# evandieren/AbstractBayesOpt.jl

Hardware: AMD Instinct MI355X
Metric: GP-update+acq-eval ms per BO step at N train pts x M candidates (lower is better)
Workload: dtype f64

## Files before the change

abstractbayesopt.jl_amd/_lib.py:

```python
import ctypes as C
import os

PKG = os.path.dirname(os.path.abspath(__file__))
LIB_PATH = os.path.join(PKG, "lib", "libabo_hip.so")
LIB_TEST_PATH = os.path.join(PKG, "lib", "libabo_hip_test.so")

ABO_OK, ABO_ENOTPD, ABO_EDIM, ABO_EINVAL, ABO_EHIP, ABO_ENOMEM = range(6)
HOST, DEVICE = 0, 1

EXPORTS = ["abo_create", "abo_set_contraction", "abo_create_grad", "abo_predict_grad", "abo_predict_grad_cov", "abo_retain", "abo_destroy", "abo_fit", "abo_append", "abo_append_grad", "abo_cand_create", "abo_cand_destroy",
           "abo_cand_refresh", "abo_cand_downdate", "abo_cand_save", "abo_cand_restore", "abo_cand_acq", "abo_cand_get", "abo_cand_point", "abo_cand_exclude", "abo_predict", "abo_acq", "abo_nlml", "abo_nlml_grad", "abo_nlml_grad_ard", "abo_lhs", "abo_score",
           "abo_get_factor", "abo_get_n", "abo_get_data", "abo_get_timings", "abo_get_prune_stats", "abo_get_prune_levels", "abo_last_error", "abo_abi_version", "abo_pool_trim",
           "abo_mgpu_create", "abo_mgpu_clone", "abo_mgpu_destroy", "abo_mgpu_info", "abo_mgpu_get", "abo_mgpu_fit",
           "abo_mgpu_predict", "abo_mgpu_acq", "abo_mgpu_acq_lhs", "abo_mgpu_append", "abo_mgpu_cand_create",
           "abo_mgpu_cand_create_lhs", "abo_mgpu_cand_refresh", "abo_mgpu_cand_destroy", "abo_mgpu_cand_acq",
           "abo_mgpu_cand_qei", "abo_refine", "abo_optimize_acquisition", "abo_mgpu_optimize_acquisition", "abo_fit_acq", "abo_mgpu_create_grad", "abo_mgpu_append_grad", "abo_mgpu_cand_get", "abo_acq_terms", "abo_acq_lhs", "abo_refine_terms",
           "abo_optimize_acquisition_terms", "abo_mgpu_optimize_acquisition_terms",
           "abo_set_qei_block", "abo_cand_qei", "abo_cand_qei_begin", "abo_cand_qei_top", "abo_cand_qei_block", "abo_cand_qei_pick",
           "abo_cand_qei_end", "abo_cand_qei_has", "abo_cand_qei_stats", "abo_mgpu_cand_qei_stats", "abo_cand_qei_eligible", "abo_fill_distance",
           "abo_update", "abo_mgpu_update", "abo_cand_qei_mc",
           "abo_paths_create", "abo_paths_destroy", "abo_paths_eval", "abo_paths_eval_cand", "abo_paths_stats_get",
           "abo_paths_append", "abo_paths_attach", "abo_paths_detach", "abo_paths_top", "abo_paths_values", "abo_paths_append_stats_get",
           "abo_score_mes", "abo_acq_mes", "abo_cand_acq_mes", "abo_refine_mes", "abo_optimize_acquisition_mes",
           "abo_loo", "abo_loo_grad", "abo_predict_cov", "abo_remove"]
TEST_EXPORTS = ["abo_test_gemm_nt", "abo_test_kappa", "abo_test_oz_plan", "abo_test_oz_contract", "abo_test_acq_grad",
                "abo_test_acq_grad_terms", "abo_test_prune_plan", "abo_test_prune_force", "abo_test_prune_levels", "abo_test_prune_plan_levels", "abo_test_prune_bounds", "abo_test_prune_mean",
                "abo_test_kappa_tail", "abo_test_prune_tail32", "abo_test_prune_reuse", "abo_test_prune_reused", "abo_test_prune_head32", "abo_test_bound_head32", "abo_test_kappa_tail32", "abo_test_prune_bound_moduli", "abo_test_prune_bound_plan", "abo_test_oz_contract_bound", "abo_test_acq_partials", "abo_test_mes_partials", "abo_test_acq_grad_mes",
                "abo_test_gemm_args", "abo_test_gemm_path", "abo_test_gemm_swz_q", "abo_test_gemm_swz_map", "abo_test_qei_pass", "abo_test_splitk_reduce",
                "abo_test_var_gemm", "abo_test_kgen", "abo_test_cand_newcol",
                "abo_test_chol_diag", "abo_test_chol_panel", "abo_test_trtri_batched", "abo_test_chol_blocked", "abo_test_trmv",
                "abo_test_nlml_terms", "abo_test_append",
                "abo_test_topk_plan", "abo_test_topk", "abo_test_prune_compact", "abo_test_prune_min_scatter", "abo_test_prune_map",
                "abo_test_finalize", "abo_test_cand_gemv", "abo_test_downdate", "abo_test_grad_cov", "abo_test_gather_points",
                "abo_test_pick_record", "abo_test_score",
                "abo_test_oz_rowscale", "abo_test_oz_quant", "abo_test_oz_gemm", "abo_test_oz_crt", "abo_test_oz_modpack", "abo_test_oz_tickets"]
TOPK_PATH_NONE, TOPK_PATH_SMALL, TOPK_PATH_SLICES, TOPK_PATH_ARGMAX, TOPK_PATH_BLOCKSORT = -1, 0, 1, 2, 3
PRUNE_REL, PRUNE_ABS, PRUNE_ABS_LOGEI = 2.0 ** -30, 2.0 ** -1022, 2.0 ** -30
GEMM_PATH_TILED, GEMM_PATH_SWIZZLED, GEMM_PATH_SMALL, GEMM_PATH_SKINNY, GEMM_PATH_SPLITK = range(5)
K_FULL, K_A_LOWER, K_A_UPPER, K_B_LOWER, K_B_UPPER = range(5)
ABI_VERSION = 7
CONTRACT_AUTO, CONTRACT_FP64, CONTRACT_INT8 = 0, 1, 2
UPDATE_SHARED, UPDATE_APPENDED, UPDATE_REFIT = 0, 1, 2
UPDATE_PATHS = {UPDATE_SHARED: "shared", UPDATE_APPENDED: "appended", UPDATE_REFIT: "refit"}
REMOVE_REMOVED, REMOVE_REFIT = 0, 1
REMOVE_PATHS = {REMOVE_REMOVED: "removed", REMOVE_REFIT: "refit"}


class AboParams(C.Structure):
    _fields_ = [("family", C.c_int32), ("device", C.c_int32), ("ell", C.c_double), ("sigma_f2", C.c_double),
                ("noise_var", C.c_double), ("mean_c", C.c_double), ("jitter", C.c_double),
                ("n_max", C.c_int64), ("chunk", C.c_int64)]


class AboTimings(C.Structure):
    _fields_ = [(n, C.c_double) for n in ("fit_kernel_matrix_ms", "fit_cholesky_ms", "fit_inverse_ms",
                                          "fit_alpha_ms", "fit_total_ms", "acq_kxz_ms", "acq_var_gemm_ms",
                                          "acq_finalize_ms", "acq_topk_ms", "acq_total_ms")] + \
               [("var_gemm_launches", C.c_int64), ("var_gemm_flop", C.c_double), ("downdate_ms", C.c_double),
                ("downdate_bytes", C.c_double), ("contraction_engine", C.c_int64), ("oz_nmod", C.c_int64)] + \
               [(n, C.c_double) for n in ("oz_prepare_ms", "oz_quant_ms", "oz_gemm_ms", "oz_crt_ms", "oz_gemm_ops", "refine_ms")] + \
               [("refine_starts", C.c_int64), ("refine_evals", C.c_int64), ("downdate_from_chain", C.c_int64),
# ... 157 lines not shown
        L.abo_test_kappa_tail.argtypes = [i32, i32, vp, vp, i64]
        L.abo_test_prune_tail32.argtypes = [i32]
        L.abo_test_prune_head32.argtypes = [i32]
        L.abo_test_prune_reuse.argtypes = [i32]
        L.abo_test_prune_reused.argtypes = [vp, C.POINTER(i32)]
        L.abo_test_bound_head32.argtypes = [vp, vp, i64, i32, vp, vp, vp, vp]
        L.abo_test_kappa_tail32.argtypes = [i32, i32, vp, vp, i64]
    L.abo_last_error.argtypes = [C.c_char_p, C.c_size_t]
    L.abo_abi_version.argtypes = []
    L.abo_pool_trim.argtypes = [i32]
    if hooks:
        L.abo_test_kappa.argtypes = [i32, i32, vp, vp, i64]
    if hooks:
        L.abo_test_oz_plan.argtypes = [i32, vp, vp, vp, vp]
    if hooks:
        L.abo_test_oz_contract.argtypes = [i32, vp, i64, i32, i32, vp, i64, i32, f64, i32, vp, i64]
        L.abo_test_oz_contract_bound.argtypes = [i32, vp, i64, i32, i32, vp, i64, i32, f64, i32, i32, vp, i64, vp]
    if hooks:
        L.abo_test_gemm_nt.argtypes = [i32, vp, vp, vp, i32, i32, i32, i64, i64, i64, f64, f64]
        L.abo_test_gemm_args.argtypes = [i32, vp, vp, vp, vp, i64, i64, i64, i64, i64, i64, i64, i64, i32, i32, i32, i32, i32, i32, f64, f64, i32, i32,
                                         vp, C.POINTER(i32)]
        L.abo_test_gemm_path.argtypes = [i32, i32, i32, i32, i32, i32, i32, i32, i32, C.POINTER(i32)]
        L.abo_test_gemm_swz_q.argtypes = [i32, i32, C.POINTER(i32)]
        L.abo_test_gemm_swz_map.argtypes = [i32, i32, i32, C.POINTER(i32), C.POINTER(i32)]
        L.abo_test_qei_pass.argtypes = [i32, vp, i64, i32, vp, i64, i64, i32, f64, vp, i64, i32, i32, i64]
        L.abo_test_splitk_reduce.argtypes = [i32, vp, i64, i64, i32, i32, i32, i32, i32, i32, vp, i64]
        L.abo_test_var_gemm.argtypes = [i32, vp, i64, i32, i32, vp, i64, i32, vp, i64, i32]
        L.abo_test_kgen.argtypes = [i32, C.POINTER(AboTestKgenArgs)]
        L.abo_test_cand_newcol.argtypes = [i32, vp, vp, vp, i64, i64, i32, i32, i32, i32, i32, i32, i32, f64, f64]
        L.abo_test_chol_diag.argtypes = [i32, vp, vp, vp, i64, i32, vp]
        L.abo_test_chol_panel.argtypes = [i32, vp, vp, vp, i64, i32, i32, i32, vp]
        L.abo_test_trtri_batched.argtypes = [i32, vp, vp, vp, i64, i32, vp]
        L.abo_test_chol_blocked.argtypes = [i32, vp, vp, vp, i64, i32, i32, i32, i32, vp]
        L.abo_test_trmv.argtypes = [i32, vp, i64, vp, vp, i32, i32]
        L.abo_test_nlml_terms.argtypes = [i32, vp, i64, vp, vp, i32, vp]
        L.abo_test_append.argtypes = [i32, C.POINTER(AboTestAppendArgs)]
        L.abo_test_topk_plan.argtypes = [i64, i32, vp]
        L.abo_test_topk.argtypes = [i32, vp, i64, i32, i64, vp, vp, C.POINTER(i32)]
        L.abo_test_prune_compact.argtypes = [i32, vp, i64, vp, f64, vp, vp]
        L.abo_test_prune_min_scatter.argtypes = [i32, vp, vp, vp, i64]
        L.abo_test_prune_map.argtypes = [i32, vp, i32, vp, i64]
        L.abo_test_finalize.argtypes = [i32, C.POINTER(AboTestFinalizeArgs)]
        L.abo_test_cand_gemv.argtypes = [i32, vp, i64, vp, i32, i64, vp]
        L.abo_test_downdate.argtypes = [i32, vp, vp, vp, i64, f64, f64]
        L.abo_test_grad_cov.argtypes = [i32, vp, vp, i64, i32, i32, i64, f64, f64, f64, vp, vp, vp, i32]
        L.abo_test_gather_points.argtypes = [i32, vp, vp, i64, i32, i32, vp]
# ... 105 lines not shown
```

abstractbayesopt.jl_amd/csrc/abo_kernels.h:

```cpp
#pragma once
#include <hip/hip_runtime.h>
#include <stdint.h>

namespace abo {

constexpr int TB = 128;
constexpr int MAX_P = 129;

inline int64_t pad_up(int64_t n, int64_t m) { return (n + m - 1) / m * m; }

enum KMode { K_FULL = 0, K_A_LOWER = 1, K_A_UPPER = 2, K_B_LOWER = 3, K_B_UPPER = 4 };

struct GemmArgs {
    const double* A;
    const double* B;
    double* C;
    double* Ct;
    int64_t lda, ldb, ldc, ldct;
    int64_t sA, sB, sC, sCt;
    int M, N, K;
    int kmode;
    int lower_only;
    int batch;
    double alpha, beta;
    const int64_t* info;
    int ksplit = 0;
    int mrows = 0;
    int swz = 0;
    int swz_g = 4;
};
hipError_t launch_gemm_nt(const GemmArgs& a, hipStream_t s);
enum GemmPath {
    GEMM_PATH_INVALID = -2,
    GEMM_PATH_NONE = -1,
    GEMM_PATH_TILED = 0,
    GEMM_PATH_SWIZZLED = 1,
    GEMM_PATH_SMALL = 2,
    GEMM_PATH_SKINNY = 3,
    GEMM_PATH_SPLITK = 4
};
inline int64_t gemm_nt_tiles(const GemmArgs& a) {
    const int64_t Tm = a.M / TB, Tn = a.N / TB;
    int64_t tiles = Tm * Tn;
    if (a.lower_only) {
        const int64_t q = Tm < Tn ? Tm : Tn;
        tiles = q * (q + 1) / 2 + (Tm - q) * Tn;
    }
    return tiles * a.batch;
}
int gemm_nt_path(const GemmArgs& a);
__host__ __device__ inline int gemm_swz_q(int L, int tiles) {
    const int per = (tiles + 7) >> 3;
    return (L & 7) * per + (L >> 3);
}
__host__ __device__ inline void gemm_swz_tile(int T, int G, int Q, int& ti, int& tj) {
    int g = (int)((sqrt(8.0 * (double)Q + 1.0) - 1.0) / (2.0 * G));
    while ((G * (g + 1)) * (G * (g + 1) + 1) / 2 <= Q) ++g;
    while ((G * g) * (G * g + 1) / 2 > Q) --g;
    int w = Q - (G * g) * (G * g + 1) / 2;
    const int r0 = G * g;
    const int R = G < T - r0 ? G : T - r0;
    if (w < R * (r0 + 1)) {
        tj = w / R;
        ti = r0 + w - tj * R;
    } else {
        w -= R * (r0 + 1);
        int c = 1;
        while (w >= R - c) { w -= R - c; ++c; }
        tj = r0 + c;
        ti = tj + w;
    }
}
hipError_t launch_splitk_reduce(const double* P, int64_t ldp, int64_t sP, int nz, int rows, int cols, int K, int ksplit, int kmode,
                                double* out, int64_t ldo, hipStream_t s);

struct VarGemmArgs {
    const double* W;
    const double* Kxz;
    double* partial;
    int64_t ldw, ldk, ldp;
    int Np, Mc;
    int nvalid;
};
hipError_t launch_var_gemm(const VarGemmArgs& a, hipStream_t s, int variant = 0);

constexpr int OZ_MAXMOD = 16;
struct OzPlan {
    int n;
    int p[OZ_MAXMOD];
    double invp[OZ_MAXMOD];
    double c26[OZ_MAXMOD];
    double s1[OZ_MAXMOD], s2[OZ_MAXMOD];
    double P1, P2, invP;
    int eP;
};
// ... 443 lines not shown
```

abstractbayesopt.jl_amd/csrc/api.hip:

```cpp
#include <hip/hip_runtime.h>

#include <algorithm>
#include <atomic>
#include <chrono>
#include <cmath>
#include <cstdarg>
#include <cstdio>
#include <cstdlib>
#include <cstring>
#include <iterator>
#include <limits>
#include <map>
#include <mutex>
#include <set>
#include <new>
#include <string>
#include <vector>

#include "abo_state.h"
#include "abo_kernels.h"
#include "kgen_core.h"

using namespace abo;

// ... 324 lines not shown
                HIPCHK(launch_potf2_diag(K, W, WT, ld, r0, info, s, trsm_ops, true));
                if (rem <= 0) break;
                HIPCHK(launch_trsm_stream(K, trsm_ops, ld, r0, rem, info, s));
                const int ncol = s0 + sw - r0 - TB;
                if (ncol > 0) {
                    GemmArgs u{};
                    u.A = K + (int64_t)(r0 + TB) * ld + r0; u.lda = ld;
                    u.B = u.A; u.ldb = ld;
                    u.C = K + (int64_t)(r0 + TB) * ld + (r0 + TB); u.ldc = ld;
                    u.M = rem; u.N = ncol; u.K = TB; u.kmode = K_FULL; u.lower_only = 1; u.batch = 1;
                    u.alpha = -1.0; u.beta = 1.0; u.info = info;
                    HIPCHK(launch_gemm_nt(u, s));
                }
            }
            const int rows = Np - s0 - sw;
            const int cols = S0 + ss - s0 - sw;
            if (rows > 0 && cols > 0) {
                GemmArgs u{};
                u.A = K + (int64_t)(s0 + sw) * ld + s0; u.lda = ld;
                u.B = u.A; u.ldb = ld;
                u.C = K + (int64_t)(s0 + sw) * ld + (s0 + sw); u.ldc = ld;
                u.M = rows; u.N = cols; u.K = sw; u.kmode = K_FULL; u.lower_only = 1; u.batch = 1;
                u.alpha = -1.0; u.beta = 1.0; u.info = info;
                HIPCHK(launch_gemm_nt(u, s));
            }
        }
        const int rest = Np - S0 - ss;
        if (rest > 0) {
            GemmArgs u{};
            u.A = K + (int64_t)(S0 + ss) * ld + S0; u.lda = ld;
            u.B = u.A; u.ldb = ld;
            u.C = K + (int64_t)(S0 + ss) * ld + (S0 + ss); u.ldc = ld;
            u.M = rest; u.N = rest; u.K = ss; u.kmode = K_FULL; u.lower_only = 1; u.batch = 1;
            u.alpha = -1.0; u.beta = 1.0; u.info = info;
            HIPCHK(launch_gemm_nt(u, s));
        }
    }
    if (split) HIPCHK(launch_trtri_diag_batched(K, W, WT, ld, Np / TB, info, s));
    return ABO_OK;
}

int32_t trinv_blocked(double* K, double* W, double* WT, double* T, int64_t ld, int Np, int64_t* info, hipStream_t s) {
    double* Tt = T;
    for (int64_t sz = TB; sz < Np; sz *= 2) {
        const int64_t two = 2 * sz;
        const int nfull = (int)(Np / two);
        const int64_t rrem = Np - (int64_t)nfull * two;
        for (int pass = 0; pass < 2; ++pass) {
            const bool ragged = pass == 1;
            if (ragged && rrem <= sz) break;
            if (!ragged && nfull == 0) continue;
            const int64_t r1 = ragged ? (int64_t)nfull * two : 0;
            const int64_t r2 = r1 + sz;
            const int64_t s2 = ragged ? rrem - sz : sz;
            const int batch = ragged ? 1 : nfull;
            const int64_t bstride = two * (ld + 1);
            double* Tp = Tt + (ragged ? (int64_t)nfull * sz * sz : 0);
            GemmArgs a{};
            a.A = WT + r1 * ld + r1; a.lda = ld; a.sA = bstride;
            a.B = K + r2 * ld + r1; a.ldb = ld; a.sB = bstride;
            a.C = Tp; a.ldc = sz; a.sC = sz * sz;
            a.M = (int)sz; a.N = (int)s2; a.K = (int)sz; a.kmode = K_A_UPPER; a.batch = batch;
            a.alpha = 1.0; a.beta = 0.0; a.info = info;
            HIPCHK(launch_gemm_nt(a, s));
            GemmArgs b{};
            b.A = W + r2 * ld + r2; b.lda = ld; b.sA = bstride;
            b.B = Tp; b.ldb = sz; b.sB = sz * sz;
            b.C = W + r2 * ld + r1; b.ldc = ld; b.sC = bstride;
            b.Ct = WT + r1 * ld + r2; b.ldct = ld; b.sCt = bstride;
            b.M = (int)s2; b.N = (int)sz; b.K = (int)s2; b.kmode = K_A_LOWER; b.batch = batch;
            b.alpha = -1.0; b.beta = 0.0; b.info = info;
            HIPCHK(launch_gemm_nt(b, s));
        }
    }
    return ABO_OK;
}

}

namespace {

int32_t factorise(abo_gp* g, double noise, int64_t* info_host) {
    hipStream_t s = g->stream;
    Storage* st = g->st;
    const int Np = (int)g->Np, N = (int)g->N;
    const int64_t ld = st->cap;
    double* K = st->K.as<double>();
    double* W = st->W.as<double>();
    double* WT = st->WT.as<double>();
    HIPCHK(g->info.ensure(sizeof(int64_t)));
    int64_t* info = g->info.as<int64_t>();

    HIPCHK(hipEventRecord(g->evs()[EV_FIT_BEGIN], s));
    const bool split = Np > TB;
// ... 2553 lines not shown
```

abstractbayesopt.jl_amd/csrc/gemm.hip:

```cpp
#include <type_traits>
#include "abo_kernels.h"
#include <cstdlib>

namespace abo {

typedef double d2_t __attribute__((ext_vector_type(2)));
typedef double d4_t __attribute__((ext_vector_type(4)));

constexpr int BM = 128, BN = 128, BK = 16;
constexpr int LDT = 20;
constexpr int TILE = BM * LDT;

__device__ __forceinline__ void tile_gload(const double* __restrict__ g, int64_t ld, int k0, d2_t (&r)[4]) {
    const int t = threadIdx.x;
    const int row = t >> 3, kk = (t & 7) * 2;
    const double* p = g + (int64_t)row * ld + k0 + kk;
#pragma unroll
    for (int q = 0; q < 4; ++q) r[q] = *reinterpret_cast<const d2_t*>(p + (int64_t)(32 * q) * ld);
}

__device__ __forceinline__ void tile_lstore(double* s, const d2_t (&r)[4]) {
    const int t = threadIdx.x;
    const int row = t >> 3, kk = (t & 7) * 2;
#pragma unroll
    for (int q = 0; q < 4; ++q) *reinterpret_cast<d2_t*>(s + (row + 32 * q) * LDT + kk) = r[q];
}

struct Frag {
    d2_t a[4], b[4];
};

__device__ __forceinline__ void frag_read(const double* ap, const double* bp, int half, Frag& f) {
#pragma unroll
    for (int i = 0; i < 4; ++i) f.a[i] = *reinterpret_cast<const d2_t*>(ap + i * 16 * LDT + half * 8);
#pragma unroll
    for (int i = 0; i < 4; ++i) f.b[i] = *reinterpret_cast<const d2_t*>(bp + i * 16 * LDT + half * 8);
}

template <int KK>
__device__ __forceinline__ void frag_mma(const Frag& f, d4_t (&acc)[4][4]) {
#pragma unroll
    for (int mi = 0; mi < 4; ++mi)
#pragma unroll
        for (int ni = 0; ni < 4; ++ni)
            acc[mi][ni] = __builtin_amdgcn_mfma_f64_16x16x4f64(f.a[mi][KK], f.b[ni][KK], acc[mi][ni], 0, 0, 0);
}

__device__ __forceinline__ void tile_loop(const double* __restrict__ Ag, int64_t lda, const double* __restrict__ Bg,
                                          int64_t ldb, int kbeg, int kend, double* smem, d4_t (&acc)[4][4]) {
    const int lane = threadIdx.x & 63, wave = threadIdx.x >> 6;
    const int wm = wave >> 1, wn = wave & 1;
    const int r16 = lane & 15, g = lane >> 4;
    const int aoff = (wm * 64 + r16) * LDT + g * 2;
    const int boff = TILE + (wn * 64 + r16) * LDT + g * 2;
    const int nk = (kend - kbeg) / BK;
    if (nk <= 0) return;
    d2_t sa[4], sb[4];
    Frag f0, f1;
    tile_gload(Ag, lda, kbeg, sa);
    tile_gload(Bg, ldb, kbeg, sb);
    tile_lstore(smem, sa);
    tile_lstore(smem + TILE, sb);
    if (nk > 1) {
        tile_gload(Ag, lda, kbeg + BK, sa);
        tile_gload(Bg, ldb, kbeg + BK, sb);
    }
    __syncthreads();
    frag_read(smem + aoff, smem + boff, 0, f0);
    int t = 0;
    {
        for (; t + 2 < nk; ++t) {
            double* cur = smem + (t & 1) * (2 * TILE);
            double* nxt = smem + ((t + 1) & 1) * (2 * TILE);
            tile_lstore(nxt, sa);
            tile_lstore(nxt + TILE, sb);
            frag_read(cur + aoff, cur + boff, 1, f1);
            tile_gload(Ag, lda, kbeg + (t + 2) * BK, sa);
            tile_gload(Bg, ldb, kbeg + (t + 2) * BK, sb);
            frag_mma<0>(f0, acc);
            frag_mma<1>(f0, acc);
#pragma unroll
            for (int i = 0; i < 8; ++i) {
                __builtin_amdgcn_sched_group_barrier(0x008, 1, 0);
                __builtin_amdgcn_sched_group_barrier(0x200, 1, 0);
            }
#pragma unroll
            for (int i = 0; i < 8; ++i) {
                __builtin_amdgcn_sched_group_barrier(0x008, 1, 0);
                __builtin_amdgcn_sched_group_barrier(0x100, 1, 0);
// ... 24 lines not shown
        frag_mma<0>(f0, acc);
        __builtin_amdgcn_sched_barrier(0);
        frag_read(cur + aoff, cur + boff, 1, f1);
        if (t + 1 < nk) {
            tile_lstore(nxt, sa);
            tile_lstore(nxt + TILE, sb);
            if (t + 2 < nk) {
                tile_gload(Ag, lda, kbeg + (t + 2) * BK, sa);
                tile_gload(Bg, ldb, kbeg + (t + 2) * BK, sb);
            }
        }
        __builtin_amdgcn_sched_barrier(0);
        frag_mma<1>(f0, acc);
        __builtin_amdgcn_sched_barrier(0);
        __syncthreads();
        if (t + 1 < nk) frag_read(nxt + aoff, nxt + boff, 0, f0);
        __builtin_amdgcn_sched_barrier(0);
        frag_mma<0>(f1, acc);
        frag_mma<1>(f1, acc);
    }
    __syncthreads();
}

__device__ __forceinline__ void acc_zero(d4_t (&acc)[4][4]) {
#pragma unroll
    for (int i = 0; i < 4; ++i)
#pragma unroll
        for (int j = 0; j < 4; ++j) acc[i][j] = d4_t{0.0, 0.0, 0.0, 0.0};
}

__global__ void __launch_bounds__(256, 2) gemm_nt_kernel(GemmArgs p) {
    __shared__ __attribute__((aligned(16))) double smem[4 * TILE];
    if (p.info != nullptr && *p.info != 0) return;
    int tj = p.kmode == K_B_LOWER ? (int)gridDim.x - 1 - (int)blockIdx.x : (int)blockIdx.x;
    int ti = p.kmode == K_A_LOWER ? (int)gridDim.y - 1 - (int)blockIdx.y : (int)blockIdx.y;
    const int bz = blockIdx.z;
    if (p.swz) {
        const int Q = gemm_swz_q((int)blockIdx.x, p.swz);
        if (Q >= p.swz) return;
        gemm_swz_tile(p.M / BM, p.swz_g, Q, ti, tj);
    }
    if (p.lower_only && tj > ti) return;
    int kbeg = 0, kend = p.K;
    if (p.kmode == K_A_LOWER) kend = min(p.K, (ti + 1) * BM);
    if (p.kmode == K_A_UPPER) kbeg = min(p.K, ti * BM);
    if (p.kmode == K_B_LOWER) kend = min(p.K, (tj + 1) * BN);
    if (p.kmode == K_B_UPPER) kbeg = min(p.K, tj * BN);
    const double* Ag = p.A + (p.ksplit ? 0 : (int64_t)bz * p.sA) + (int64_t)ti * BM * p.lda;
    const double* Bg = p.B + (p.ksplit ? 0 : (int64_t)bz * p.sB) + (int64_t)tj * BN * p.ldb;
    if (p.ksplit) {
        kbeg = max(kbeg, bz * p.ksplit);
        kend = min(kend, (bz + 1) * p.ksplit);
        if (kbeg >= kend) return;
    }
    d4_t acc[4][4];
    acc_zero(acc);
    tile_loop(Ag, p.lda, Bg, p.ldb, kbeg, kend, smem, acc);

    const int lane = threadIdx.x & 63, wave = threadIdx.x >> 6;
    const int wm = wave >> 1, wn = wave & 1;
    const int r16 = lane & 15, g = lane >> 4;
    double* Cg = p.C + (int64_t)bz * p.sC;
    double* Ctg = p.Ct ? p.Ct + (int64_t)bz * p.sCt : nullptr;
#pragma unroll
    for (int mi = 0; mi < 4; ++mi)
#pragma unroll
        for (int ni = 0; ni < 4; ++ni)
#pragma unroll
            for (int r = 0; r < 4; ++r) {
                const int64_t row = (int64_t)ti * BM + wm * 64 + mi * 16 + g + 4 * r;
                const int64_t col = (int64_t)tj * BN + wn * 64 + ni * 16 + r16;
                double v = p.alpha * acc[mi][ni][r];
                if (p.beta != 0.0) v += p.beta * Cg[row * p.ldc + col];
                Cg[row * p.ldc + col] = v;
                if (Ctg) Ctg[col * p.ldct + row] = v;
            }
}

__global__ void __launch_bounds__(256) gemm_nt_small_kernel(GemmArgs p) {
    if (p.info != nullptr && *p.info != 0) return;
    const int sj = blockIdx.x, si = blockIdx.y, bz = blockIdx.z;
    const int ti = si >> 2, tj = sj >> 2;
    if (p.lower_only && tj > ti) return;
    int kbeg = 0, kend = p.K;
    if (p.kmode == K_A_LOWER) kend = min(p.K, (ti + 1) * BM);
    if (p.kmode == K_A_UPPER) kbeg = min(p.K, ti * BM);
    if (p.kmode == K_B_LOWER) kend = min(p.K, (tj + 1) * BN);
    if (p.kmode == K_B_UPPER) kbeg = min(p.K, tj * BN);
    const int lane = threadIdx.x & 63, wave = threadIdx.x >> 6;
    const int wm = wave >> 1, wn = wave & 1;
    const int r16 = lane & 15, g = lane >> 4;
    const double* Ap = p.A + (int64_t)bz * p.sA + (int64_t)(si * 32 + wm * 16 + r16) * p.lda + 2 * g;
    const double* Bp = p.B + (int64_t)bz * p.sB + (int64_t)(sj * 32 + wn * 16 + r16) * p.ldb + 2 * g;
    double* Cg = p.C + (int64_t)bz * p.sC;
    double* Ctg = p.Ct ? p.Ct + (int64_t)bz * p.sCt : nullptr;
    double cin[4] = {0.0, 0.0, 0.0, 0.0};
    if (p.beta != 0.0) {
#pragma unroll
        for (int r = 0; r < 4; ++r)
            cin[r] = Cg[((int64_t)si * 32 + wm * 16 + g + 4 * r) * p.ldc + (int64_t)sj * 32 + wn * 16 + r16];
    }
    d4_t acc = {0.0, 0.0, 0.0, 0.0};
    for (int k = kbeg; k < kend; k += 128) {
        d2_t a[16], b[16];
#pragma unroll
        for (int q = 0; q < 16; ++q) {
            a[q] = *reinterpret_cast<const d2_t*>(Ap + k + 8 * q);
            b[q] = *reinterpret_cast<const d2_t*>(Bp + k + 8 * q);
        }
#pragma unroll
        for (int q = 0; q < 16; ++q) {
            acc = __builtin_amdgcn_mfma_f64_16x16x4f64(a[q][0], b[q][0], acc, 0, 0, 0);
            acc = __builtin_amdgcn_mfma_f64_16x16x4f64(a[q][1], b[q][1], acc, 0, 0, 0);
        }
    }
#pragma unroll
    for (int r = 0; r < 4; ++r) {
        const int64_t row = (int64_t)si * 32 + wm * 16 + g + 4 * r;
        const int64_t col = (int64_t)sj * 32 + wn * 16 + r16;
        double v = p.alpha * acc[r];
        if (p.beta != 0.0) v += p.beta * cin[r];
        Cg[row * p.ldc + col] = v;
        if (Ctg) Ctg[col * p.ldct + row] = v;
    }
}

template <int RG>
__global__ void __launch_bounds__(256) gemm_skinny_kernel(GemmArgs p) {
    if (p.info != nullptr && *p.info != 0) return;
    const int tj = p.kmode == K_B_LOWER ? (int)gridDim.x - 1 - (int)blockIdx.x : (int)blockIdx.x, bz = blockIdx.z;
    int kbeg = 0, kend = p.K;
    if (p.kmode == K_B_LOWER) kend = min(p.K, (tj + 1) * BN);
    if (p.kmode == K_B_UPPER) kbeg = min(p.K, tj * BN);
    kbeg = max(kbeg, bz * p.ksplit);
    kend = min(kend, (bz + 1) * p.ksplit);
    if (kbeg >= kend) return;
    const int lane = threadIdx.x & 63, wave = threadIdx.x >> 6;
    const int r16 = lane & 15, g = lane >> 4;
    const double* Bp = p.B + (int64_t)(tj * BN + wave * 32 + r16) * p.ldb + 2 * g;
    const double* Ap = p.A + (int64_t)r16 * p.lda + 2 * g;
    d4_t acc[RG][2];
#pragma unroll
    for (int q = 0; q < RG; ++q) { acc[q][0] = d4_t{0.0, 0.0, 0.0, 0.0}; acc[q][1] = d4_t{0.0, 0.0, 0.0, 0.0}; }
    for (int k = kbeg; k < kend; k += 64) {
        d2_t b0[8], b1[8], a[RG][8];
#pragma unroll
        for (int q = 0; q < 8; ++q) {
// ... 114 lines not shown
            C[row * ldc + row0 + r16] = alpha * acc[r][e];
        }
}

hipError_t launch_qei_pass(const double* A, int64_t lda, int rows16, const double* B, int64_t ldb, int64_t nB, int K, double alpha,
                           double* C, int64_t ldc, hipStream_t s, int kmode, int ksplit, int64_t sC) {
    if (nB <= 0) return hipSuccess;
    if (rows16 < 16 || rows16 > 64 || rows16 % 16 || nB % 128 || K <= 0 || K % 128 || (lda & 1) || (ldb & 1)) return hipErrorInvalidValue;
    if (kmode != K_FULL && kmode != K_B_LOWER && kmode != K_B_UPPER) return hipErrorInvalidValue;
    if (ksplit <= 0) ksplit = K;
    if (ksplit % 128) return hipErrorInvalidValue;
    dim3 gridd((unsigned)(nB / 64), 1, (unsigned)((K + ksplit - 1) / ksplit));
#define QP_LAUNCH(RG_) hipLaunchKernelGGL((qei_passd_kernel<RG_, 2>), gridd, dim3(256), 0, s, A, lda, B, ldb, C, ldc, K, alpha, kmode, ksplit, sC)
    switch (rows16 / 16) {
        case 1: QP_LAUNCH(1); break;
        case 2: QP_LAUNCH(2); break;
        case 3: QP_LAUNCH(3); break;
        default: QP_LAUNCH(4); break;
    }
#undef QP_LAUNCH
    return hipGetLastError();
}

int gemm_nt_path(const GemmArgs& a) {
    if (a.M <= 0 || a.N <= 0 || a.batch <= 0) return GEMM_PATH_NONE;
    if (a.ksplit) {
        if (a.batch != 1 || a.beta != 0.0 || a.ksplit % 128 != 0 || a.Ct) return GEMM_PATH_INVALID;
        return a.mrows >= 16 && a.mrows <= 64 && a.mrows % 16 == 0 && a.M == BM ? GEMM_PATH_SKINNY : GEMM_PATH_SPLITK;
    }
    const char* fe = getenv("ABO_GEMM_SMALL");
    const int force = fe ? atoi(fe) : -1;
    const bool small = force >= 0 ? force == 1 : gemm_nt_tiles(a) <= 64;
    const bool in_place = a.C == a.A || a.C == a.B;
    if (small && !in_place && a.K % 128 == 0) return GEMM_PATH_SMALL;
    if (a.lower_only && a.kmode == K_FULL && a.M == a.N && a.batch == 1 && a.M / BM >= 16 && !getenv("ABO_GEMM_NO_SWIZZLE")) return GEMM_PATH_SWIZZLED;
    return GEMM_PATH_TILED;
}

hipError_t launch_gemm_nt(const GemmArgs& a, hipStream_t s) {
    switch (gemm_nt_path(a)) {
        case GEMM_PATH_NONE: return hipSuccess;
        case GEMM_PATH_INVALID: return hipErrorInvalidValue;
        case GEMM_PATH_SKINNY: {
            dim3 grid(a.N / BN, a.M / BM, (a.K + a.ksplit - 1) / a.ksplit);
            switch (a.mrows / 16) {
                case 1: hipLaunchKernelGGL((gemm_skinny_kernel<1>), grid, dim3(256), 0, s, a); break;
                case 2: hipLaunchKernelGGL((gemm_skinny_kernel<2>), grid, dim3(256), 0, s, a); break;
                case 3: hipLaunchKernelGGL((gemm_skinny_kernel<3>), grid, dim3(256), 0, s, a); break;
                default: hipLaunchKernelGGL((gemm_skinny_kernel<4>), grid, dim3(256), 0, s, a); break;
            }
            break;
        }
        case GEMM_PATH_SPLITK: {
            dim3 grid(a.N / BN, a.M / BM, (a.K + a.ksplit - 1) / a.ksplit);
            hipLaunchKernelGGL(gemm_nt_kernel, grid, dim3(256), 0, s, a);
            break;
        }
        case GEMM_PATH_SMALL: {
            dim3 grid(a.N / 32, a.M / 32, a.batch);
            hipLaunchKernelGGL(gemm_nt_small_kernel, grid, dim3(256), 0, s, a);
            break;
        }
        case GEMM_PATH_SWIZZLED: {
// ... 248 lines not shown
```

include/abo_hip.h:

```cpp
#ifndef ABO_HIP_H
#define ABO_HIP_H

#include <stddef.h>
#include <stdint.h>

#ifdef __cplusplus
extern "C" {
#endif

#define ABO_ABI_VERSION 7

enum {
    ABO_OK = 0,
    ABO_ENOTPD = 1,
    ABO_EDIM = 2,
    ABO_EINVAL = 3,
    ABO_EHIP = 4,
    ABO_ENOMEM = 5
};

enum { ABO_KERNEL_SE = 0, ABO_KERNEL_MATERN52 = 1, ABO_KERNEL_MATERN72 = 2, ABO_KERNEL_MATERN32 = 3 };

enum {
    ABO_ACQ_EI = 0,
// ... 279 lines not shown
int32_t abo_test_oz_plan(int32_t n, int32_t* p, double* tables, double* scal, int32_t* eP);
int32_t abo_test_oz_contract(int32_t device, const double* W, int64_t ldw, int32_t Np, int32_t nvalid, const double* Kxz, int64_t ldk,
                             int32_t Mc, double kmax, int32_t nmod, double* partial, int64_t ldp);
int32_t abo_test_oz_contract_bound(int32_t device, const double* W, int64_t ldw, int32_t Np, int32_t nvalid, const double* Kxz, int64_t ldk,
                                   int32_t Mc, double kmax, int32_t nmod_b, int32_t rblocks, double* partial, int64_t ldp, double* delta);
int32_t abo_test_acq_grad(abo_gp* gp, int32_t kind, double p0, double best_y, const double* Z, int64_t M, int32_t d, double* f,
                          double* grad);
int32_t abo_test_acq_grad_terms(abo_gp* gp, const abo_acq_term* terms, int32_t nterms, const double* Z, int64_t M, int32_t d,
                                double* f, double* grad);
int32_t abo_test_acq_partials(int32_t device, const double* mu, const double* var, int64_t M, int32_t kind, double p0, double best_y,
                              double* f, double* dmu, double* dvar);
int32_t abo_test_mes_partials(int32_t device, const double* mu, const double* var, int64_t M, const double* ystar, int32_t S, double* f,
                              double* dmu, double* dvar);
int32_t abo_test_acq_grad_mes(abo_gp* gp, const double* ystar, int32_t S, const double* Z, int64_t M, int32_t d, double* f, double* grad);
int32_t abo_test_kappa(int32_t device, int32_t family, const double* d2, double* out, int64_t n);
int32_t abo_test_gemm_nt(int32_t device, const double* A, const double* B, double* C, int32_t M,
                         int32_t N, int32_t K, int64_t lda, int64_t ldb, int64_t ldc, double alpha,
                         double beta);
#define ABO_GEMM_PATH_TILED 0
#define ABO_GEMM_PATH_SWIZZLED 1
#define ABO_GEMM_PATH_SMALL 2
#define ABO_GEMM_PATH_SKINNY 3
#define ABO_GEMM_PATH_SPLITK 4
int32_t abo_test_gemm_args(int32_t device, const double* A, const double* B, double* C, double* Ct, int64_t lda, int64_t ldb, int64_t ldc,
                           int64_t ldct, int64_t sA, int64_t sB, int64_t sC, int64_t sCt, int32_t M, int32_t N, int32_t K, int32_t kmode,
                           int32_t lower_only, int32_t batch, double alpha, double beta, int32_t ksplit, int32_t mrows, const int64_t* info,
                           int32_t* path);
int32_t abo_test_gemm_path(int32_t M, int32_t N, int32_t K, int32_t kmode, int32_t lower_only, int32_t batch, int32_t ksplit,
                           int32_t mrows, int32_t in_place, int32_t* path);
int32_t abo_test_gemm_swz_q(int32_t tiles, int32_t L, int32_t* Q);
int32_t abo_test_gemm_swz_map(int32_t T, int32_t G, int32_t Q, int32_t* ti, int32_t* tj);
int32_t abo_test_qei_pass(int32_t device, const double* A, int64_t lda, int32_t rows16, const double* B, int64_t ldb, int64_t nB, int32_t K,
                          double alpha, double* C, int64_t ldc, int32_t kmode, int32_t ksplit, int64_t sC);
int32_t abo_test_splitk_reduce(int32_t device, const double* P, int64_t ldp, int64_t sP, int32_t nz, int32_t rows, int32_t cols, int32_t K,
                               int32_t ksplit, int32_t kmode, double* out, int64_t ldo);
int32_t abo_test_var_gemm(int32_t device, const double* W, int64_t ldw, int32_t Np, int32_t nvalid, const double* Kxz, int64_t ldk, int32_t Mc,
                          double* partial, int64_t ldp, int32_t variant);
typedef struct abo_test_kgen_args {
    const double* Xs; const double* Z; const double* alpha; double* Kout; double* mu;
    int64_t ldk, M, j0;
    int32_t Mc, N, Np, d, dp, family;
    double s, sigma_f2;
    const double* mean_vec;
    int32_t pt, pc, point_major, dlogell, rvalid, n_mean;
    int8_t* res; int64_t res_ld, res_plane; int32_t* res_bad;
    int32_t res_n, res_sK, res_ktg, res_kmax;
} abo_test_kgen_args;
int32_t abo_test_kgen(int32_t device, const abo_test_kgen_args* args);
int32_t abo_test_cand_newcol(int32_t device, const double* Xs, const double* Z, double* Kzx, int64_t ld, int64_t M, int32_t col, int32_t grad,
                             int32_t pt, int32_t q, int32_t d, int32_t dp, int32_t family, double s, double sigma_f2);
int32_t abo_test_chol_diag(int32_t device, double* K, double* W, double* WT, int64_t ld, int32_t r0, int64_t* info);
int32_t abo_test_chol_panel(int32_t device, double* K, double* W, double* WT, int64_t ld, int32_t r0, int32_t nrows, int32_t zero_rows,
                            int64_t* info);
int32_t abo_test_trtri_batched(int32_t device, double* K, double* W, double* WT, int64_t ld, int32_t nblocks, int64_t* info);
// ... 72 lines not shown
```

Before: 19.62.

## Add persistent GEMM kernel with cross-tile prefetch for Cholesky and trtri updates

Adds a persistent-workgroup GEMM path that launches about two workgroups per CU. Each workgroup walks a static tile sequence, in snake order for triangular k-ranges, and prefetches the next tile's first K-slab while it stores the current one. Leftover tail tiles go to a small-piece kernel split into 16 sub-blocks. The blocked Cholesky trailing updates and the batched triangular-inverse GEMMs now request this path, aiming to cut launch and tail-wave imbalance. The tile-to-position mapping adds complexity, and fixed slots may hurt if the load is uneven.

```diff
diff --git a/abstractbayesopt.jl_amd/_lib.py b/abstractbayesopt.jl_amd/_lib.py
--- a/abstractbayesopt.jl_amd/_lib.py
+++ b/abstractbayesopt.jl_amd/_lib.py
@@ -26,7 +26,7 @@
 TEST_EXPORTS = ["abo_test_gemm_nt", "abo_test_kappa", "abo_test_oz_plan", "abo_test_oz_contract", "abo_test_acq_grad",
                 "abo_test_acq_grad_terms", "abo_test_prune_plan", "abo_test_prune_force", "abo_test_prune_levels", "abo_test_prune_plan_levels", "abo_test_prune_bounds", "abo_test_prune_mean",
                 "abo_test_kappa_tail", "abo_test_prune_tail32", "abo_test_prune_reuse", "abo_test_prune_reused", "abo_test_prune_head32", "abo_test_bound_head32", "abo_test_kappa_tail32", "abo_test_prune_bound_moduli", "abo_test_prune_bound_plan", "abo_test_oz_contract_bound", "abo_test_acq_partials", "abo_test_mes_partials", "abo_test_acq_grad_mes",
-                "abo_test_gemm_args", "abo_test_gemm_path", "abo_test_gemm_swz_q", "abo_test_gemm_swz_map", "abo_test_qei_pass", "abo_test_splitk_reduce",
+                "abo_test_gemm_args", "abo_test_gemm_path", "abo_test_gemm_swz_q", "abo_test_gemm_swz_map", "abo_test_gemm_persist_map", "abo_test_qei_pass", "abo_test_splitk_reduce",
                 "abo_test_var_gemm", "abo_test_kgen", "abo_test_cand_newcol",
                 "abo_test_chol_diag", "abo_test_chol_panel", "abo_test_trtri_batched", "abo_test_chol_blocked", "abo_test_trmv",
                 "abo_test_nlml_terms", "abo_test_append",
@@ -36,7 +36,7 @@
                 "abo_test_oz_rowscale", "abo_test_oz_quant", "abo_test_oz_gemm", "abo_test_oz_crt", "abo_test_oz_modpack", "abo_test_oz_tickets"]
 TOPK_PATH_NONE, TOPK_PATH_SMALL, TOPK_PATH_SLICES, TOPK_PATH_ARGMAX, TOPK_PATH_BLOCKSORT = -1, 0, 1, 2, 3
 PRUNE_REL, PRUNE_ABS, PRUNE_ABS_LOGEI = 2.0 ** -30, 2.0 ** -1022, 2.0 ** -30
-GEMM_PATH_TILED, GEMM_PATH_SWIZZLED, GEMM_PATH_SMALL, GEMM_PATH_SKINNY, GEMM_PATH_SPLITK = range(5)
+GEMM_PATH_TILED, GEMM_PATH_SWIZZLED, GEMM_PATH_SMALL, GEMM_PATH_SKINNY, GEMM_PATH_SPLITK, GEMM_PATH_PERSIST = range(6)
 K_FULL, K_A_LOWER, K_A_UPPER, K_B_LOWER, K_B_UPPER = range(5)
 ABI_VERSION = 7
 CONTRACT_AUTO, CONTRACT_FP64, CONTRACT_INT8 = 0, 1, 2
@@ -240,6 +240,7 @@
                                          vp, C.POINTER(i32)]
         L.abo_test_gemm_path.argtypes = [i32, i32, i32, i32, i32, i32, i32, i32, i32, C.POINTER(i32)]
         L.abo_test_gemm_swz_q.argtypes = [i32, i32, C.POINTER(i32)]
+        L.abo_test_gemm_persist_map.argtypes = [i32, i32, i32, i32, i32, i32, vp, i64, C.POINTER(i64), C.POINTER(i32)]
         L.abo_test_gemm_swz_map.argtypes = [i32, i32, i32, C.POINTER(i32), C.POINTER(i32)]
         L.abo_test_qei_pass.argtypes = [i32, vp, i64, i32, vp, i64, i64, i32, f64, vp, i64, i32, i32, i64]
         L.abo_test_splitk_reduce.argtypes = [i32, vp, i64, i64, i32, i32, i32, i32, i32, i32, vp, i64]
diff --git a/abstractbayesopt.jl_amd/csrc/abo_kernels.h b/abstractbayesopt.jl_amd/csrc/abo_kernels.h
--- a/abstractbayesopt.jl_amd/csrc/abo_kernels.h
+++ b/abstractbayesopt.jl_amd/csrc/abo_kernels.h
@@ -28,6 +28,8 @@
     int mrows = 0;
     int swz = 0;
     int swz_g = 4;
+    int persist = 0;
+    int p_slots = 0, p_whole = 0, p_snake = 0;
 };
 hipError_t launch_gemm_nt(const GemmArgs& a, hipStream_t s);
 enum GemmPath {
@@ -37,7 +39,8 @@
     GEMM_PATH_SWIZZLED = 1,
     GEMM_PATH_SMALL = 2,
     GEMM_PATH_SKINNY = 3,
-    GEMM_PATH_SPLITK = 4
+    GEMM_PATH_SPLITK = 4,
+    GEMM_PATH_PERSIST = 5
 };
 inline int64_t gemm_nt_tiles(const GemmArgs& a) {
     const int64_t Tm = a.M / TB, Tn = a.N / TB;
@@ -71,6 +74,66 @@
         ti = tj + w;
     }
 }
+__host__ __device__ inline int gemm_seq_per_batch(const GemmArgs& a) {
+    const int Tm = a.M / TB, Tn = a.N / TB;
+    if (!a.lower_only) return Tm * Tn;
+    const int q = Tm < Tn ? Tm : Tn;
+    return q * (q + 1) / 2 + (Tm - q) * Tn;
+}
+__host__ __device__ inline int gemm_seq_len(const GemmArgs& a) {
+    return a.swz ? (a.swz + 7) / 8 * 8 : gemm_seq_per_batch(a) * a.batch;
+}
+__host__ __device__ inline bool gemm_seq_tile(const GemmArgs& a, int pos, int& ti, int& tj, int& bz) {
+    const int Tm = a.M / TB, Tn = a.N / TB;
+    bz = 0;
+    if (a.swz) {
+        const int Q = gemm_swz_q(pos, a.swz);
+        if (Q >= a.swz) return false;
+        gemm_swz_tile(Tm, a.swz_g, Q, ti, tj);
+        return true;
+    }
+    const int per = gemm_seq_per_batch(a);
+    bz = pos / per;
+    if (bz >= a.batch) return false;
+    int w = pos - bz * per;
+    if (a.lower_only) {
+        const int q = Tm < Tn ? Tm : Tn, tri = q * (q + 1) / 2;
+        if (w < tri) {
+            ti = (int)((sqrt(8.0 * (double)w + 1.0) - 1.0) / 2.0);
+            while ((ti + 1) * (ti + 2) / 2 <= w) ++ti;
+            while (ti * (ti + 1) / 2 > w) --ti;
+            tj = w - ti * (ti + 1) / 2;
+        } else {
+            w -= tri;
+            ti = q + w / Tn;
+            tj = w - (ti - q) * Tn;
+        }
+        return true;
+    }
+    const int y = w / Tn, x = w - y * Tn;
+    tj = a.kmode == K_B_LOWER ? Tn - 1 - x : x;
+    ti = a.kmode == K_A_LOWER ? Tm - 1 - y : y;
+    return true;
+}
+__host__ __device__ inline int gemm_persist_pos(int w, int r, int slots, int snake) {
+    return r * slots + ((snake && (r & 1)) ? slots - 1 - w : w);
+}
+constexpr int GEMM_PERSIST_TAIL_DIV = 16;
+struct GemmPersistPlan { int slots, len, whole, wgs, rounds, snake; };
+__host__ __device__ inline GemmPersistPlan gemm_persist_plan(const GemmArgs& a, int slots, int tail_max, int under_max) {
+    GemmPersistPlan pl{};
+    pl.slots = slots;
+    pl.len = gemm_seq_len(a);
+    pl.snake = a.kmode != K_FULL;
+    const int tiles = a.swz ? a.swz : pl.len;
+    const int left = pl.len % slots;
+    if (pl.len < slots) pl.whole = tiles <= under_max ? 0 : pl.len;
+    else pl.whole = left <= tail_max ? pl.len - left : pl.len;
+    pl.wgs = pl.whole < slots ? pl.whole : slots;
+    pl.rounds = (pl.whole + slots - 1) / slots;
+    return pl;
+}
+GemmPersistPlan gemm_persist_setup(const GemmArgs& a, int slots, GemmArgs& b);
 hipError_t launch_splitk_reduce(const double* P, int64_t ldp, int64_t sP, int nz, int rows, int cols, int K, int ksplit, int kmode,
                                 double* out, int64_t ldo, hipStream_t s);
 
diff --git a/abstractbayesopt.jl_amd/csrc/api.hip b/abstractbayesopt.jl_amd/csrc/api.hip
--- a/abstractbayesopt.jl_amd/csrc/api.hip
+++ b/abstractbayesopt.jl_amd/csrc/api.hip
@@ -370,6 +370,7 @@
                 u.C = K + (int64_t)(s0 + sw) * ld + (s0 + sw); u.ldc = ld;
                 u.M = rows; u.N = cols; u.K = sw; u.kmode = K_FULL; u.lower_only = 1; u.batch = 1;
                 u.alpha = -1.0; u.beta = 1.0; u.info = info;
+                u.persist = 1;
                 HIPCHK(launch_gemm_nt(u, s));
             }
         }
@@ -381,6 +382,7 @@
             u.C = K + (int64_t)(S0 + ss) * ld + (S0 + ss); u.ldc = ld;
             u.M = rest; u.N = rest; u.K = ss; u.kmode = K_FULL; u.lower_only = 1; u.batch = 1;
             u.alpha = -1.0; u.beta = 1.0; u.info = info;
+            u.persist = 1;
             HIPCHK(launch_gemm_nt(u, s));
         }
     }
@@ -410,6 +412,7 @@
             a.C = Tp; a.ldc = sz; a.sC = sz * sz;
             a.M = (int)sz; a.N = (int)s2; a.K = (int)sz; a.kmode = K_A_UPPER; a.batch = batch;
             a.alpha = 1.0; a.beta = 0.0; a.info = info;
+            a.persist = gemm_nt_tiles(a) > 64;
             HIPCHK(launch_gemm_nt(a, s));
             GemmArgs b{};
             b.A = W + r2 * ld + r2; b.lda = ld; b.sA = bstride;
@@ -418,6 +421,7 @@
             b.Ct = WT + r1 * ld + r2; b.ldct = ld; b.sCt = bstride;
             b.M = (int)s2; b.N = (int)sz; b.K = (int)s2; b.kmode = K_A_LOWER; b.batch = batch;
             b.alpha = -1.0; b.beta = 0.0; b.info = info;
+            b.persist = gemm_nt_tiles(b) > 64;
             HIPCHK(launch_gemm_nt(b, s));
         }
     }
diff --git a/abstractbayesopt.jl_amd/csrc/gemm.hip b/abstractbayesopt.jl_amd/csrc/gemm.hip
--- a/abstractbayesopt.jl_amd/csrc/gemm.hip
+++ b/abstractbayesopt.jl_amd/csrc/gemm.hip
@@ -46,25 +46,26 @@
             acc[mi][ni] = __builtin_amdgcn_mfma_f64_16x16x4f64(f.a[mi][KK], f.b[ni][KK], acc[mi][ni], 0, 0, 0);
 }
 
-__device__ __forceinline__ void tile_loop(const double* __restrict__ Ag, int64_t lda, const double* __restrict__ Bg,
-                                          int64_t ldb, int kbeg, int kend, double* smem, d4_t (&acc)[4][4]) {
+__device__ __forceinline__ void tile_head_load(const double* __restrict__ Ag, int64_t lda, const double* __restrict__ Bg, int64_t ldb,
+                                               int k0, d2_t (&sa)[4], d2_t (&sb)[4]) {
+    tile_gload(Ag, lda, k0, sa);
+    tile_gload(Bg, ldb, k0, sb);
+}
+__device__ __forceinline__ void tile_head_stage(const double* __restrict__ Ag, int64_t lda, const double* __restrict__ Bg, int64_t ldb,
+                                                int kbeg, int nk, double* smem, d2_t (&sa)[4], d2_t (&sb)[4]) {
+    tile_lstore(smem, sa);
+    tile_lstore(smem + TILE, sb);
+    if (nk > 1) tile_head_load(Ag, lda, Bg, ldb, kbeg + BK, sa, sb);
+}
+
+__device__ __forceinline__ void tile_body(const double* __restrict__ Ag, int64_t lda, const double* __restrict__ Bg, int64_t ldb,
+                                          int kbeg, int nk, double* smem, d2_t (&sa)[4], d2_t (&sb)[4], d4_t (&acc)[4][4]) {
     const int lane = threadIdx.x & 63, wave = threadIdx.x >> 6;
     const int wm = wave >> 1, wn = wave & 1;
     const int r16 = lane & 15, g = lane >> 4;
     const int aoff = (wm * 64 + r16) * LDT + g * 2;
     const int boff = TILE + (wn * 64 + r16) * LDT + g * 2;
-    const int nk = (kend - kbeg) / BK;
-    if (nk <= 0) return;
-    d2_t sa[4], sb[4];
     Frag f0, f1;
-    tile_gload(Ag, lda, kbeg, sa);
-    tile_gload(Bg, ldb, kbeg, sb);
-    tile_lstore(smem, sa);
-    tile_lstore(smem + TILE, sb);
-    if (nk > 1) {
-        tile_gload(Ag, lda, kbeg + BK, sa);
-        tile_gload(Bg, ldb, kbeg + BK, sb);
-    }
     __syncthreads();
     frag_read(smem + aoff, smem + boff, 0, f0);
     int t = 0;
@@ -135,11 +136,51 @@
     __syncthreads();
 }
 
+__device__ __forceinline__ void tile_loop(const double* __restrict__ Ag, int64_t lda, const double* __restrict__ Bg,
+                                          int64_t ldb, int kbeg, int kend, double* smem, d4_t (&acc)[4][4]) {
+    const int nk = (kend - kbeg) / BK;
+    if (nk <= 0) return;
+    d2_t sa[4], sb[4];
+    tile_head_load(Ag, lda, Bg, ldb, kbeg, sa, sb);
+    tile_head_stage(Ag, lda, Bg, ldb, kbeg, nk, smem, sa, sb);
+    tile_body(Ag, lda, Bg, ldb, kbeg, nk, smem, sa, sb, acc);
+}
+
 __device__ __forceinline__ void acc_zero(d4_t (&acc)[4][4]) {
 #pragma unroll
     for (int i = 0; i < 4; ++i)
 #pragma unroll
         for (int j = 0; j < 4; ++j) acc[i][j] = d4_t{0.0, 0.0, 0.0, 0.0};
+}
+
+__device__ __forceinline__ void tile_krange(const GemmArgs& p, int ti, int tj, int& kbeg, int& kend) {
+    kbeg = 0; kend = p.K;
+    if (p.kmode == K_A_LOWER) kend = min(p.K, (ti + 1) * BM);
+    if (p.kmode == K_A_UPPER) kbeg = min(p.K, ti * BM);
+    if (p.kmode == K_B_LOWER) kend = min(p.K, (tj + 1) * BN);
+    if (p.kmode == K_B_UPPER) kbeg = min(p.K, tj * BN);
+}
+
+template <int MI0, int MI1>
+__device__ __forceinline__ void tile_store(const GemmArgs& p, int ti, int tj, int bz, const d4_t (&acc)[4][4]) {
+    const int lane = threadIdx.x & 63, wave = threadIdx.x >> 6;
+    const int wm = wave >> 1, wn = wave & 1;
+    const int r16 = lane & 15, g = lane >> 4;
+    double* Cg = p.C + (int64_t)bz * p.sC;
+    double* Ctg = p.Ct ? p.Ct + (int64_t)bz * p.sCt : nullptr;
+#pragma unroll
+    for (int mi = MI0; mi < MI1; ++mi)
+#pragma unroll
+        for (int ni = 0; ni < 4; ++ni)
+#pragma unroll
+            for (int r = 0; r < 4; ++r) {
+                const int64_t row = (int64_t)ti * BM + wm * 64 + mi * 16 + g + 4 * r;
+                const int64_t col = (int64_t)tj * BN + wn * 64 + ni * 16 + r16;
+                double v = p.alpha * acc[mi][ni][r];
+                if (p.beta != 0.0) v += p.beta * Cg[row * p.ldc + col];
+                Cg[row * p.ldc + col] = v;
+                if (Ctg) Ctg[col * p.ldct + row] = v;
+            }
 }
 
 __global__ void __launch_bounds__(256, 2) gemm_nt_kernel(GemmArgs p) {
@@ -154,11 +195,8 @@
         gemm_swz_tile(p.M / BM, p.swz_g, Q, ti, tj);
     }
     if (p.lower_only && tj > ti) return;
-    int kbeg = 0, kend = p.K;
-    if (p.kmode == K_A_LOWER) kend = min(p.K, (ti + 1) * BM);
-    if (p.kmode == K_A_UPPER) kbeg = min(p.K, ti * BM);
-    if (p.kmode == K_B_LOWER) kend = min(p.K, (tj + 1) * BN);
-    if (p.kmode == K_B_UPPER) kbeg = min(p.K, tj * BN);
+    int kbeg, kend;
+    tile_krange(p, ti, tj, kbeg, kend);
     const double* Ag = p.A + (p.ksplit ? 0 : (int64_t)bz * p.sA) + (int64_t)ti * BM * p.lda;
     const double* Bg = p.B + (p.ksplit ? 0 : (int64_t)bz * p.sB) + (int64_t)tj * BN * p.ldb;
     if (p.ksplit) {
@@ -170,36 +208,56 @@
     acc_zero(acc);
     tile_loop(Ag, p.lda, Bg, p.ldb, kbeg, kend, smem, acc);
 
-    const int lane = threadIdx.x & 63, wave = threadIdx.x >> 6;
-    const int wm = wave >> 1, wn = wave & 1;
-    const int r16 = lane & 15, g = lane >> 4;
-    double* Cg = p.C + (int64_t)bz * p.sC;
-    double* Ctg = p.Ct ? p.Ct + (int64_t)bz * p.sCt : nullptr;
-#pragma unroll
-    for (int mi = 0; mi < 4; ++mi)
-#pragma unroll
-        for (int ni = 0; ni < 4; ++ni)
-#pragma unroll
-            for (int r = 0; r < 4; ++r) {
-                const int64_t row = (int64_t)ti * BM + wm * 64 + mi * 16 + g + 4 * r;
-                const int64_t col = (int64_t)tj * BN + wn * 64 + ni * 16 + r16;
-                double v = p.alpha * acc[mi][ni][r];
-                if (p.beta != 0.0) v += p.beta * Cg[row * p.ldc + col];
-                Cg[row * p.ldc + col] = v;
-                if (Ctg) Ctg[col * p.ldct + row] = v;
-            }
-}
-
-__global__ void __launch_bounds__(256) gemm_nt_small_kernel(GemmArgs p) {
+    tile_store<0, 4>(p, ti, tj, bz, acc);
+}
+
+struct PTile { const double *Ag, *Bg; int ti, tj, bz, kbeg, nk; };
+__device__ __forceinline__ bool persist_next(const GemmArgs& p, int& r, int rounds, PTile& t) {
+    for (; r < rounds; ++r) {
+        const int pos = gemm_persist_pos((int)blockIdx.x, r, p.p_slots, p.p_snake);
+        if (pos >= p.p_whole || !gemm_seq_tile(p, pos, t.ti, t.tj, t.bz)) continue;
+        int kend;
+        tile_krange(p, t.ti, t.tj, t.kbeg, kend);
+        t.nk = (kend - t.kbeg) / BK;
+        t.Ag = p.A + (int64_t)t.bz * p.sA + (int64_t)t.ti * BM * p.lda;
+        t.Bg = p.B + (int64_t)t.bz * p.sB + (int64_t)t.tj * BN * p.ldb;
+        ++r;
+        return true;
+    }
+    return false;
+}
+
+__global__ void __launch_bounds__(256, 2) gemm_nt_persist_kernel(GemmArgs p) {
+    __shared__ __attribute__((aligned(16))) double smem[4 * TILE];
     if (p.info != nullptr && *p.info != 0) return;
-    const int sj = blockIdx.x, si = blockIdx.y, bz = blockIdx.z;
+    const int rounds = (p.p_whole + p.p_slots - 1) / p.p_slots;
+    int r = 0;
+    PTile cur, nxt;
+    bool have = persist_next(p, r, rounds, cur);
+    d2_t sa[4], sb[4];
+    if (have && cur.nk > 0) {
+        tile_head_load(cur.Ag, p.lda, cur.Bg, p.ldb, cur.kbeg, sa, sb);
+        tile_head_stage(cur.Ag, p.lda, cur.Bg, p.ldb, cur.kbeg, cur.nk, smem, sa, sb);
+    }
+    while (have) {
+        d4_t acc[4][4];
+        acc_zero(acc);
+        if (cur.nk > 0) tile_body(cur.Ag, p.lda, cur.Bg, p.ldb, cur.kbeg, cur.nk, smem, sa, sb, acc);
+        have = persist_next(p, r, rounds, nxt);
+        tile_store<0, 4>(p, cur.ti, cur.tj, cur.bz, acc);
+        if (have && nxt.nk > 0) {
+            tile_head_load(nxt.Ag, p.lda, nxt.Bg, p.ldb, nxt.kbeg, sa, sb);
+            tile_head_stage(nxt.Ag, p.lda, nxt.Bg, p.ldb, nxt.kbeg, nxt.nk, smem, sa, sb);
+        }
+        cur = nxt;
+    }
+}
+
+__device__ __forceinline__ void small_piece(const GemmArgs& p, int si, int sj, int bz) {
     const int ti = si >> 2, tj = sj >> 2;
     if (p.lower_only && tj > ti) return;
-    int kbeg = 0, kend = p.K;
-    if (p.kmode == K_A_LOWER) kend = min(p.K, (ti + 1) * BM);
-    if (p.kmode == K_A_UPPER) kbeg = min(p.K, ti * BM);
-    if (p.kmode == K_B_LOWER) kend = min(p.K, (tj + 1) * BN);
-    if (p.kmode == K_B_UPPER) kbeg = min(p.K, tj * BN);
+    int kbeg, kend;
+    tile_krange(p, ti, tj, kbeg, kend);
     const int lane = threadIdx.x & 63, wave = threadIdx.x >> 6;
     const int wm = wave >> 1, wn = wave & 1;
     const int r16 = lane & 15, g = lane >> 4;
@@ -236,6 +294,19 @@
         Cg[row * p.ldc + col] = v;
         if (Ctg) Ctg[col * p.ldct + row] = v;
     }
+}
+
+__global__ void __launch_bounds__(256) gemm_nt_small_kernel(GemmArgs p) {
+    if (p.info != nullptr && *p.info != 0) return;
+    small_piece(p, blockIdx.y, blockIdx.x, blockIdx.z);
+}
+
+__global__ void __launch_bounds__(256) gemm_nt_pieces_kernel(GemmArgs p) {
+    if (p.info != nullptr && *p.info != 0) return;
+    const int u = blockIdx.x, piece = u & 15;
+    int ti, tj, bz;
+    if (!gemm_seq_tile(p, p.p_whole + (u >> 4), ti, tj, bz)) return;
+    small_piece(p, 4 * ti + (piece >> 2), 4 * tj + (piece & 3), bz);
 }
 
 template <int RG>
@@ -396,23 +467,61 @@
     return hipGetLastError();
 }
 
+static bool gemm_swizzles(const GemmArgs& a) {
+    return a.lower_only && a.kmode == K_FULL && a.M == a.N && a.batch == 1 && a.M / BM >= 16 && !getenv("ABO_GEMM_NO_SWIZZLE");
+}
+
 int gemm_nt_path(const GemmArgs& a) {
     if (a.M <= 0 || a.N <= 0 || a.batch <= 0) return GEMM_PATH_NONE;
     if (a.ksplit) {
-        if (a.batch != 1 || a.beta != 0.0 || a.ksplit % 128 != 0 || a.Ct) return GEMM_PATH_INVALID;
+        if (a.batch != 1 || a.beta != 0.0 || a.ksplit % 128 != 0 || a.Ct || a.persist) return GEMM_PATH_INVALID;
         return a.mrows >= 16 && a.mrows <= 64 && a.mrows % 16 == 0 && a.M == BM ? GEMM_PATH_SKINNY : GEMM_PATH_SPLITK;
     }
     const char* fe = getenv("ABO_GEMM_SMALL");
     const int force = fe ? atoi(fe) : -1;
     const bool small = force >= 0 ? force == 1 : gemm_nt_tiles(a) <= 64;
     const bool in_place = a.C == a.A || a.C == a.B;
+    const char* pe = getenv("ABO_GEMM_PERSIST");
+    const bool persist = a.persist && !(pe && atoi(pe) == 0);
+    if (persist && (in_place || a.K % 128 != 0)) return GEMM_PATH_INVALID;
     if (small && !in_place && a.K % 128 == 0) return GEMM_PATH_SMALL;
-    if (a.lower_only && a.kmode == K_FULL && a.M == a.N && a.batch == 1 && a.M / BM >= 16 && !getenv("ABO_GEMM_NO_SWIZZLE")) return GEMM_PATH_SWIZZLED;
+    if (persist) return GEMM_PATH_PERSIST;
+    if (gemm_swizzles(a)) return GEMM_PATH_SWIZZLED;
     return GEMM_PATH_TILED;
+}
+
+static int gemm_persist_device_slots() {
+    static int cached[64] = {};
+    int dev = 0;
+    if (hipGetDevice(&dev) != hipSuccess || dev < 0 || dev >= 64) return 0;
+    if (!cached[dev]) {
+        int cus = 0;
+        if (hipDeviceGetAttribute(&cus, hipDeviceAttributeMultiprocessorCount, dev) != hipSuccess || cus <= 0) return 0;
+        cached[dev] = 2 * cus;
+    }
+    return cached[dev];
+}
+
+GemmPersistPlan gemm_persist_setup(const GemmArgs& a, int slots, GemmArgs& b) {
+    b = a;
+    if (gemm_swizzles(a)) { b.swz = (int)gemm_nt_tiles(a); b.swz_g = 4; }
+    const GemmPersistPlan pl = gemm_persist_plan(b, slots, (slots + GEMM_PERSIST_TAIL_DIV - 1) / GEMM_PERSIST_TAIL_DIV, (slots + 3) / 4 - 1);
+    b.p_slots = pl.slots; b.p_whole = pl.whole; b.p_snake = pl.snake;
+    return pl;
 }
 
 hipError_t launch_gemm_nt(const GemmArgs& a, hipStream_t s) {
     switch (gemm_nt_path(a)) {
+        case GEMM_PATH_PERSIST: {
+            const char* se = getenv("ABO_GEMM_PERSIST_SLOTS");
+            const int slots = se && atoi(se) > 0 ? atoi(se) : gemm_persist_device_slots();
+            if (slots <= 0 || gemm_nt_tiles(a) > (int64_t)1 << 30) return hipErrorInvalidValue;
+            GemmArgs b;
+            const GemmPersistPlan pl = gemm_persist_setup(a, slots, b);
+            if (pl.wgs > 0) hipLaunchKernelGGL(gemm_nt_persist_kernel, dim3((unsigned)pl.wgs), dim3(256), 0, s, b);
+            if (pl.len > pl.whole) hipLaunchKernelGGL(gemm_nt_pieces_kernel, dim3((unsigned)(16 * (pl.len - pl.whole))), dim3(256), 0, s, b);
+            break;
+        }
         case GEMM_PATH_NONE: return hipSuccess;
         case GEMM_PATH_INVALID: return hipErrorInvalidValue;
         case GEMM_PATH_SKINNY: {
diff --git a/include/abo_hip.h b/include/abo_hip.h
--- a/include/abo_hip.h
+++ b/include/abo_hip.h
@@ -325,6 +325,7 @@
 #define ABO_GEMM_PATH_SMALL 2
 #define ABO_GEMM_PATH_SKINNY 3
 #define ABO_GEMM_PATH_SPLITK 4
+#define ABO_GEMM_PATH_PERSIST 5
 int32_t abo_test_gemm_args(int32_t device, const double* A, const double* B, double* C, double* Ct, int64_t lda, int64_t ldb, int64_t ldc,
                            int64_t ldct, int64_t sA, int64_t sB, int64_t sC, int64_t sCt, int32_t M, int32_t N, int32_t K, int32_t kmode,
                            int32_t lower_only, int32_t batch, double alpha, double beta, int32_t ksplit, int32_t mrows, const int64_t* info,
@@ -333,6 +334,8 @@
                            int32_t mrows, int32_t in_place, int32_t* path);
 int32_t abo_test_gemm_swz_q(int32_t tiles, int32_t L, int32_t* Q);
 int32_t abo_test_gemm_swz_map(int32_t T, int32_t G, int32_t Q, int32_t* ti, int32_t* tj);
+int32_t abo_test_gemm_persist_map(int32_t M, int32_t N, int32_t kmode, int32_t lower_only, int32_t batch, int32_t slots, int32_t* rec,
+                                  int64_t cap, int64_t* count, int32_t* wgs);
 int32_t abo_test_qei_pass(int32_t device, const double* A, int64_t lda, int32_t rows16, const double* B, int64_t ldb, int64_t nB, int32_t K,
                           double alpha, double* C, int64_t ldc, int32_t kmode, int32_t ksplit, int64_t sC);
 int32_t abo_test_splitk_reduce(int32_t device, const double* P, int64_t ldp, int64_t sP, int32_t nz, int32_t rows, int32_t cols, int32_t K,
```

After: 19.46, median of 6. Within noise of the previous version (-0.8%).
